# cmusphinx/pocketsphinx

Measured on NVIDIA H100. Metric: frames/sec senone-eval+Viterbi, higher is better.
Workload: dtype f32->i16/i32

## Files before the change

include/psb200.h:

```cpp
#ifndef PSB200_H
#define PSB200_H

#include <stddef.h>
#include <stdint.h>

#ifdef __cplusplus
extern "C" {
#endif

#define PSB_ABI_VERSION 2

typedef enum psb_status_e {
    PSB_OK = 0,
    PSB_ERR_ARG = -1,
    PSB_ERR_CUDA = -2,
    PSB_ERR_NOMEM = -3,
    PSB_ERR_STATE = -4
} psb_status_t;

enum { PSB_KIND_PTM = 0, PSB_KIND_SEMI = 1, PSB_KIND_MS = 2 };

#define PSB_MAX_FEAT 8
#define PSB_MAX_TOPN 8
#define PSB_HMM_MAX_NSTATE 5
// ... 34 lines not shown
int psb_scorer_reset(psb_scorer_t *s);
int psb_scorer_set_frame_idx(psb_scorer_t *s, int32_t frame_idx);
int32_t psb_scorer_get_frame_idx(const psb_scorer_t *s);
int psb_scorer_frame_eval(psb_scorer_t *s, int16_t *senscr, const uint8_t *senone_active,
                          int32_t n_senone_active, const float *const *feat, int32_t frame,
                          int32_t compallsen);

typedef struct psb_batch_s psb_batch_t;

int psb_batch_create(psb_model_t *m, int32_t max_utts, int64_t max_frames, psb_batch_t **out);
void psb_batch_free(psb_batch_t *b);
int psb_batch_score_host(psb_batch_t *b, const float *feats, const int32_t *utt_off,
                         int32_t n_utt, int16_t *senscr);
int psb_batch_score_device(psb_batch_t *b, const float *d_feats, const int32_t *utt_off,
                           int32_t n_utt, int16_t *d_senscr);
int psb_batch_sync(psb_batch_t *b);
int16_t *psb_batch_senscr_device(psb_batch_t *b);
int psb_batch_last_kernel_ms(psb_batch_t *b, float *out3);
int psb_batch_event_record(psb_batch_t *b, int slot);
int psb_batch_event_elapsed_ms(psb_batch_t *b, float *ms);
int psb_batch_tc_check(psb_batch_t *b, float *ratio, int32_t *max_candidates, int64_t *stats4);
#define PSB_TC_N_COUNTERS 15
int psb_batch_tc_counters(psb_batch_t *b, int64_t *out, int32_t n);
#define PSB_MS_PLAN_N 14
int psb_batch_ms_plan(psb_batch_t *b, int64_t total_frames, int64_t *out, int32_t n);
#define PSB_TM_PLAN_N 5
int psb_batch_tm_plan(psb_batch_t *b, int64_t total_frames, int64_t *out, int32_t n);
int psb_batch_get_topn(psb_batch_t *b, int32_t *rec, int64_t n_frames);

typedef struct psb_hmm_s {
    void *ctx;
    int32_t score[PSB_HMM_MAX_NSTATE];
    int32_t history[PSB_HMM_MAX_NSTATE];
    int32_t out_score;
    int32_t out_history;
    uint16_t ssid;
    uint16_t senid[PSB_HMM_MAX_NSTATE];
    int32_t bestscore;
    int16_t tmatid;
    int32_t frame;
    uint8_t mpx;
    uint8_t n_emit_state;
} psb_hmm_t;

typedef struct psb_hmmctx_s psb_hmmctx_t;

// ... 268 lines not shown
```

pocketsphinx_b200/_lib.py:

```python
import ctypes as C
import os

HERE = os.path.dirname(os.path.abspath(__file__))
LIB_PATH = os.path.join(HERE, "libpsb200.so")

MAX_FEAT = 8


class PsbError(RuntimeError):
    pass


class ModelDesc(C.Structure):
    _fields_ = [("kind", C.c_int32), ("n_sen", C.c_int32), ("n_mgau", C.c_int32), ("n_feat", C.c_int32),
                ("n_density", C.c_int32), ("topn", C.c_int32), ("featlen", C.c_int32 * MAX_FEAT),
                ("ds_ratio", C.c_int32), ("aw", C.c_int32), ("logadd_ms_size", C.c_int32),
                ("logadd_ms_zero", C.c_int32), ("on_device", C.c_int32),
                ("mean", C.c_void_p), ("var", C.c_void_p), ("det", C.c_void_p), ("mixw", C.c_void_p),
                ("mixw_cb", C.c_void_p), ("sen2cb", C.c_void_p), ("logadd8", C.c_void_p),
                ("logadd_ms", C.c_void_p), ("topn_beam", C.c_void_p), ("fixed_point", C.c_int32)]


_VP, _I32, _I64 = C.c_void_p, C.c_int32, C.c_int64
class FeDesc(C.Structure):
# ... 56 lines not shown
    ("psb_scorer_get_frame_idx", _I32, [_VP]),
    ("psb_scorer_frame_eval", C.c_int, [_VP, _VP, _VP, _I32, _VP, _I32, _I32]),
    ("psb_batch_create", C.c_int, [_VP, _I32, _I64, C.POINTER(_VP)]),
    ("psb_batch_free", None, [_VP]),
    ("psb_batch_score_host", C.c_int, [_VP, _VP, _VP, _I32, _VP]),
    ("psb_batch_score_device", C.c_int, [_VP, _VP, _VP, _I32, _VP]),
    ("psb_batch_sync", C.c_int, [_VP]),
    ("psb_batch_senscr_device", _VP, [_VP]),
    ("psb_batch_last_kernel_ms", C.c_int, [_VP, _VP]),
    ("psb_batch_get_topn", C.c_int, [_VP, _VP, _I64]),
    ("psb_batch_event_record", C.c_int, [_VP, C.c_int]),
    ("psb_batch_event_elapsed_ms", C.c_int, [_VP, _VP]),
    ("psb_hmmctx_create", C.c_int, [_I32, _VP, _I32, _VP, _I32, _I32, C.c_int, C.POINTER(_VP)]),
    ("psb_hmmctx_free", None, [_VP]),
    ("psb_hmm_vit_eval_batch", C.c_int, [_VP, _VP, _I32, _VP, _VP]),
    ("psb_hmm_vit_eval_ptrs", C.c_int, [_VP, _VP, _I32, _VP, _VP]),
    ("psb_hmmset_create", C.c_int, [_VP, C.c_int64, _I32, C.POINTER(_VP)]),
    ("psb_hmmset_free", None, [_VP]),
    ("psb_hmmset_upload", C.c_int, [_VP, _VP, C.c_int64, _VP, _I32]),
    ("psb_hmmset_download", C.c_int, [_VP, _VP]),
    ("psb_hmmset_eval_frames_device", C.c_int, [_VP, _VP, _VP, _VP, _I32, _VP, C.POINTER(C.c_float)]),
    ("psb_batch_tc_check", C.c_int, [_VP, C.POINTER(C.c_float), C.POINTER(C.c_int32), _VP]),
    ("psb_batch_tc_counters", C.c_int, [_VP, _VP, _I32]),
    ("psb_batch_ms_plan", C.c_int, [_VP, _I64, _VP, _I32]),
    ("psb_batch_tm_plan", C.c_int, [_VP, _I64, _VP, _I32]),
    ("psb_hmmset_use_batch_stream", C.c_int, [_VP, _VP]),
    ("psb_hmmset_snapshot", C.c_int, [_VP]),
    ("psb_hmmset_restore", C.c_int, [_VP]),
    ("psb_hmmset_sweep_device", C.c_int, [_VP, _VP, _I64, _VP, _VP, _I32, _VP, C.POINTER(C.c_float)]),
    ("psb_hmmset_sweep_beam_device", C.c_int, [_VP, _VP, _I64, _VP, _VP, _I32, _I32, _I32, _I32, _VP, _VP, C.POINTER(C.c_float)]),
    ("psb_hmmset_eval_host", C.c_int, [_VP, _VP, _VP]),
    ("psb_allphone_batch_device", C.c_int, [_VP, _VP, _VP, _I32, _I32, _VP, _VP, _VP, _VP, _I32, _I32, _I32, _I32, _VP, _I32, _VP]),
    ("psb_allphone_lm_batch_device", C.c_int, [_VP, _VP, _VP, _I32, _I32, _VP, _VP, _VP, _VP, _I32, _I32, _I32, _I32, _VP, _VP, _VP, _VP, _I32, _VP]),
    ("psb_allphone_net_batch_device", C.c_int, [_VP, _VP, _VP, _I32, _I32, _VP, _VP, _VP, _VP, _VP, _I32, _I32, _I32, _I32, _I32, _VP, _VP, _I32, _VP, _VP, _I32, _VP]),
    ("psb_kws_batch_device", C.c_int, [_VP, _VP, _VP, _I32, _I32, _VP, _VP, _I32, _VP, _VP, _VP, _VP, _I32, _I32, _VP, _I32, _VP]),
    ("psb_fsg_batch_device", C.c_int, [_VP, C.POINTER(FsgDesc), _VP, _VP, _I32, _VP, _I32, _VP]),
    ("psb_ngram_fwdtree_batch_device", C.c_int, [_VP, C.POINTER(NgramDesc), _VP, _VP, _I32, _VP, _I32, _VP, _I32, _VP, _I32, _VP, _VP]),
    ("psb_ngram_fwdflat_batch_device", C.c_int, [_VP, C.POINTER(NgramDesc), _VP, _VP, _I32, _VP, _I32, _VP, _VP, _I32, _VP, _I32, _VP, _VP]),
    ("psb_selftest_block_scan", C.c_int, [C.c_int, _VP, _I32, _VP]),
    ("psb_fsg_find_exit", C.c_int, [_VP, _I32, _VP, _I32, _I32, _I32, _I32, _VP, _VP]),
    ("psb_fsg_backtrace", _I32, [_VP, _I32, _VP, _I32, _I32, _VP, _I32]),
    ("psb_ngram_find_exit", C.c_int, [_VP, _I32, _VP, _I32, _I32, _VP, _VP]),
    ("psb_ngram_backtrace", _I32, [_VP, _I32, _I32, _VP, _I32]),
    ("psb_ngram_segments", _I32, [C.POINTER(NgramDesc), _VP, _I32, _VP, _I32, _I32, C.c_float, _VP, _I32]),
    ("psb_ngram_two_pass_batch_device", C.c_int, [_VP, C.POINTER(NgramDesc), _VP, _VP, _I32, _VP, _I32, _I32, _I32, _VP, _I32, _VP, _I32,
                                                   _VP, _VP, _VP]),
# ... 72 lines not shown
```

pocketsphinx_b200/csrc/psb_ptm_tc.cu:

```cuda
#include "psb_gau.cuh"
#include "psb_internal.cuh"

#include <algorithm>
#include <cmath>
#include <cstring>

namespace {

constexpr int TC_ROWS = 128;
constexpr int TC_K = 32;
constexpr int TC_CAP = 18;
constexpr float TC_ERR = 1.0f / 262144.f;

enum {
    ST_ROWS, ST_FILTER_ALONE, ST_EXACT_DIST, ST_TIE_FLAGS,
    ST_OVER_CAP,
    ST_LANE_OVER,
    ST_FALLBACK_LISTED, ST_FALLBACK_ALL,
    ST_SPLIT,
    ST_FAIL_GAP, ST_FAIL_STRADDLE, ST_FAIL_SIGN, ST_FAIL_SAT,
    ST_N
};
constexpr size_t TC_CHECK_BYTES = 16 + 8 * ST_N;

__device__ __forceinline__ float to_tf32(float x)
{
    unsigned r;
    asm("cvt.rna.tf32.f32 %0, %1;" : "=r"(r) : "f"(x));
    return __uint_as_float(r);
}

struct Top5 {
    int s[5];
    unsigned c;
    int c4;
    int n;
};

__device__ __forceinline__ void top5_insert(Top5 &t, int s, int c)
{
    int p = 0;
#pragma unroll
    for (int j = 0; j < 5; ++j) p += (j < t.n && t.s[j] >= s) ? 1 : 0;
    if (p >= 5) return;
#pragma unroll
    for (int j = 4; j >= 1; --j)
        if (j > p) t.s[j] = t.s[j - 1];
#pragma unroll
    for (int j = 0; j < 5; ++j)
        if (j == p) t.s[j] = s;
    if (p < 4) {
        const unsigned lowmask = p == 0 ? 0u : (0xffffffffu >> (32 - 8 * p));
        t.c4 = (int)(t.c >> 24);
        t.c = (t.c & lowmask) | ((unsigned)c << (8 * p)) | ((t.c << 8) & ~(lowmask | (0xffu << (8 * p))));
    }
    else
        t.c4 = c;
    if (t.n < 5) ++t.n;
}

constexpr int WG_ROWS = 64;
constexpr int WG_SLOTS = (TC_CAP + 1) * WG_ROWS * 4;
constexpr int WG_EXTRA = WG_SLOTS * 8 + WG_ROWS * 4 * 4 + WG_ROWS * 4 + 2 * WG_ROWS * 4 + WG_ROWS * 20;

__device__ __forceinline__ uint64_t wgmma_desc(const void *p, unsigned lbo_bytes, unsigned sbo_bytes)
{
    const uint64_t a = (uint64_t)(((unsigned)__cvta_generic_to_shared(p) >> 4) & 0x3fffu);
    return a | ((uint64_t)((lbo_bytes >> 4) & 0x3fffu) << 16) | ((uint64_t)((sbo_bytes >> 4) & 0x3fffu) << 32);
}

template <int R>
__device__ __forceinline__ void wgmma_fence_regs(float (&d)[R])
{
#pragma unroll
    for (int i = 0; i < R; ++i) asm volatile("" : "+f"(d[i])::"memory");
}

__device__ __forceinline__ void warpgroup_bar(int id) { asm volatile("bar.sync %0, 128;" ::"r"(id) : "memory"); }

template <int N>
struct Wgmma;
#define PSB_ACC8(i) "+f"(d[i]), "+f"(d[i + 1]), "+f"(d[i + 2]), "+f"(d[i + 3]), "+f"(d[i + 4]), "+f"(d[i + 5]), "+f"(d[i + 6]), "+f"(d[i + 7])
template <> struct Wgmma<64> {
    static __device__ __forceinline__ void mma(float (&d)[32], uint64_t a, uint64_t b, int accumulate)
    {
        asm volatile("{\n.reg .pred p;\nsetp.ne.b32 p, %34, 0;\nwgmma.mma_async.sync.aligned.m64n64k8.f32.tf32.tf32 {"
// ... 14 lines not shown
        "}, %64, %65, p, 1, 1;\n}\n"
        : PSB_ACC8(0), PSB_ACC8(8), PSB_ACC8(16), PSB_ACC8(24), PSB_ACC8(32), PSB_ACC8(40), PSB_ACC8(48), PSB_ACC8(56)
        : "l"(a), "l"(b), "r"(accumulate));
    }
};
template <> struct Wgmma<256> {
    static __device__ __forceinline__ void mma(float (&d)[128], uint64_t a, uint64_t b, int accumulate)
    {
        asm volatile("{\n.reg .pred p;\nsetp.ne.b32 p, %130, 0;\nwgmma.mma_async.sync.aligned.m64n256k8.f32.tf32.tf32 {"
        "%0,%1,%2,%3,%4,%5,%6,%7,%8,%9,%10,%11,%12,%13,%14,%15,%16,%17,%18,%19,%20,%21,%22,%23,%24,%25,%26,%27,%28,%29,"
        "%30,%31,%32,%33,%34,%35,%36,%37,%38,%39,%40,%41,%42,%43,%44,%45,%46,%47,%48,%49,%50,%51,%52,%53,%54,%55,%56,"
        "%57,%58,%59,%60,%61,%62,%63,%64,%65,%66,%67,%68,%69,%70,%71,%72,%73,%74,%75,%76,%77,%78,%79,%80,%81,%82,%83,"
        "%84,%85,%86,%87,%88,%89,%90,%91,%92,%93,%94,%95,%96,%97,%98,%99,%100,%101,%102,%103,%104,%105,%106,%107,%108,"
        "%109,%110,%111,%112,%113,%114,%115,%116,%117,%118,%119,%120,%121,%122,%123,%124,%125,%126,%127"
        "}, %128, %129, p, 1, 1;\n}\n"
        : PSB_ACC8(0), PSB_ACC8(8), PSB_ACC8(16), PSB_ACC8(24), PSB_ACC8(32), PSB_ACC8(40), PSB_ACC8(48), PSB_ACC8(56),
          PSB_ACC8(64), PSB_ACC8(72), PSB_ACC8(80), PSB_ACC8(88), PSB_ACC8(96), PSB_ACC8(104), PSB_ACC8(112),
          PSB_ACC8(120)
        : "l"(a), "l"(b), "r"(accumulate));
    }
};
#undef PSB_ACC8

template <int FL, int ND, bool CHECK>
__global__ void __launch_bounds__(2 * 128, 1)
ptm_wgmma_kernel(const float *__restrict__ feats, long long total, int D, const int32_t *__restrict__ featoff,
                 const int32_t *__restrict__ klist, const float *__restrict__ wumma, const float *__restrict__ cen,
                 const float *__restrict__ bnd, const float *__restrict__ rec, const size_t *__restrict__ rec_off,
                 int4 *__restrict__ out, unsigned *__restrict__ flags, long long flag_words, int K, int n_feat,
                 int tiles_per_cta, uint4 *__restrict__ items, unsigned *__restrict__ n_items, unsigned item_cap,
                 float *__restrict__ check, unsigned long long *__restrict__ stats)
{
    constexpr int RF = (1 + 2 * FL + 3) / 4 * 4;
    constexpr int NTL = ND / 8;
    constexpr int NPG = NTL / 8;
    constexpr unsigned FULL = 0xffffffffu;
    static_assert(2 * FL + 1 <= TC_K && (ND == 64 || ND == 128 || ND == 256), "shape");
    extern __shared__ __align__(128) unsigned char wg_smem[];
    const int tid = threadIdx.x, wg = tid >> 7, t = tid & 127, warp = t >> 5, lane = tid & 31;
    float *sW = reinterpret_cast<float *>(wg_smem);
    float *sX = sW + 2 * 8 * ND * 4 + wg * (2 * 8 * WG_ROWS * 4);
    unsigned char *ex = wg_smem + (size_t)2 * 8 * ND * 16 + 2 * (2 * 8 * WG_ROWS * 16) + (size_t)wg * WG_EXTRA;
    float2 *Pv = reinterpret_cast<float2 *>(ex);
    unsigned *Pm = reinterpret_cast<unsigned *>(Pv + WG_SLOTS);
    float *thrs = reinterpret_cast<float *>(Pm + WG_ROWS * 4);
    float *epsr = thrs + WG_ROWS;
    unsigned *Lc = reinterpret_cast<unsigned *>(epsr + 2 * WG_ROWS);

    const int k = klist[blockIdx.x];
    const int f = k % n_feat;
    {
        const float4 *src = reinterpret_cast<const float4 *>(wumma + (size_t)k * 2 * 8 * ND * 4);
        float4 *dst = reinterpret_cast<float4 *>(sW);
        for (int i = tid; i < 2 * 8 * ND; i += 2 * 128) dst[i] = src[i];
    }
    __syncthreads();
    const float *m = cen + (size_t)k * 16, *bb = bnd + (size_t)k * 32;
    const float *rc = rec + rec_off[k];
    const int r = t & (WG_ROWS - 1), half = t >> 6;
    const int g = lane >> 2, q4 = lane & 3;
    const int ra = warp * 16 + g, rb = ra + 8;

    float xn[FL];
    auto fetch = [&](long long row) {
        const float *p = feats + (row < total ? row : 0) * D + featoff[f];
#pragma unroll
        for (int j = 0; j < FL; ++j) xn[j] = row < total ? p[j] : 0.f;
    };
    auto prepare = [&](float *eps) {
        float v[TC_K];
        float S = bb[2 * FL];
#pragma unroll
        for (int j = 0; j < FL; ++j) {
            const float y = __fsub_rn(xn[j], m[j]);
            const float y2 = __fmul_rn(y, y);
            v[j] = y2;
            v[FL + j] = y;
            if (half == 0) {
                S = __fadd_ru(S, __fmul_ru(bb[j], y2));
                S = __fadd_ru(S, __fmul_ru(bb[FL + j], fabsf(y)));
            }
        }
        v[2 * FL] = 1.0f;
#pragma unroll
        for (int j = 2 * FL + 1; j < TC_K; ++j) v[j] = 0.f;
#pragma unroll
        for (int kc = 0; kc < 8; ++kc) {
            if ((kc & 1) != half) continue;
            float4 h, l;
            h.x = to_tf32(v[4 * kc]); h.y = to_tf32(v[4 * kc + 1]); h.z = to_tf32(v[4 * kc + 2]); h.w = to_tf32(v[4 * kc + 3]);
            l.x = to_tf32(__fsub_rn(v[4 * kc], h.x)); l.y = to_tf32(__fsub_rn(v[4 * kc + 1], h.y));
            l.z = to_tf32(__fsub_rn(v[4 * kc + 2], h.z)); l.w = to_tf32(__fsub_rn(v[4 * kc + 3], h.w));
            reinterpret_cast<float4 *>(sX)[kc * WG_ROWS + r] = h;
            reinterpret_cast<float4 *>(sX)[(8 + kc) * WG_ROWS + r] = l;
        }
        if (half == 0) eps[r] = __fadd_ru(__fmul_ru(S, TC_ERR), 2.0f);
        asm volatile("fence.proxy.async.shared::cta;" ::: "memory");
        warpgroup_bar(1 + wg);
    };
    float acc[ND / 2];
    auto gemm = [&]() {
#pragma unroll
        for (int i = 0; i < ND / 2; ++i) acc[i] = 0.f;
        wgmma_fence_regs(acc);
        asm volatile("wgmma.fence.sync.aligned;" ::: "memory");
#pragma unroll
        for (int pass = 0; pass < 3; ++pass) {
            const int ha = pass == 0 ? 1 : 0, hb = pass == 1 ? 1 : 0;
#pragma unroll
            for (int ks = 0; ks < 4; ++ks) {
                const uint64_t ad = wgmma_desc(sX + (size_t)(ha * 8 + 2 * ks) * WG_ROWS * 4, WG_ROWS * 16, 128);
                const uint64_t bd = wgmma_desc(sW + (size_t)(hb * 8 + 2 * ks) * ND * 4, ND * 16, 128);
                Wgmma<ND>::mma(acc, ad, bd, (pass | ks) ? 1 : 0);
            }
        }
        asm volatile("wgmma.commit_group.sync.aligned;" ::: "memory");
    };

    auto resolve = [&](const long long row0, const float *eps) {
        const int rr = t >> 1, h = t & 1;
        const long long row = row0 + rr;
        const bool valid = row < total;
        unsigned char *lb = reinterpret_cast<unsigned char *>(Lc + rr * 5);
        float a[5] = {-INFINITY, -INFINITY, -INFINITY, -INFINITY, -INFINITY};
        int c[5] = {0, 0, 0, 0, 0};
        int nl = 0;
        bool over = false;
        {
            const float thr = thrs[rr];
            auto cand = [&](float v, int col) {
                const bool p = v >= thr;
                if (p && nl < TC_CAP) lb[h ? TC_CAP - 1 - nl : nl] = (unsigned char)col;
                nl += p ? 1 : 0;
                v = p ? v : -INFINITY;
#pragma unroll
                for (int j = 0; j < 5; ++j) {
                    const bool s = v > a[j];
                    const float tv = a[j];
                    const int tc = c[j];
                    a[j] = s ? v : tv; c[j] = s ? col : tc;
                    v = s ? tv : v; col = s ? tc : col;
                }
            };
            unsigned m0 = Pm[rr * 4 + 2 * h], m1 = Pm[rr * 4 + 2 * h + 1];
            over = __popc(m0) > TC_CAP || __popc(m1) > TC_CAP;
            int j0 = 0, j1 = 0;
            while ((m0 | m1) != 0u) {
                const bool first = m0 != 0u;
                const unsigned msk = first ? m0 : m1;
                const int i = __ffs(msk) - 1, q = 2 * h + (first ? 0 : 1), j = first ? j0 : j1;
                const float2 v = Pv[j * WG_ROWS * 4 + rr * 4 + q];
                cand(v.x, 8 * i + 2 * q);
                cand(v.y, 8 * i + 2 * q + 1);
                if (first) { m0 = ++j0 < TC_CAP ? m0 & (m0 - 1u) : 0u; }
                else { m1 = ++j1 < TC_CAP ? m1 & (m1 - 1u) : 0u; }
            }
        }
        const int n1 = __shfl_xor_sync(FULL, nl, 1), n = nl + n1;
        over = __shfl_xor_sync(FULL, (int)over, 1) != 0 || over;
        {
            float b[5];
            int bc[5];
#pragma unroll
            for (int j = 0; j < 5; ++j) { b[j] = __shfl_xor_sync(FULL, a[j], 1); bc[j] = __shfl_xor_sync(FULL, c[j], 1); }
#pragma unroll
// ... 27 lines not shown
                    if (n > TC_CAP) atomicAdd(stats + ST_OVER_CAP, 1ull);
                    if (over) atomicAdd(stats + ST_LANE_OVER, 1ull);
                    if (listed) {
                        if (!gap_ok) atomicAdd(stats + ST_FAIL_GAP, 1ull);
                        if (!straddle_ok) atomicAdd(stats + ST_FAIL_STRADDLE, 1ull);
                        if (!sign_ok) atomicAdd(stats + ST_FAIL_SIGN, 1ull);
                        if (!sat_ok) atomicAdd(stats + ST_FAIL_SAT, 1ull);
                    }
                }
                if (certain) {
                    unsigned cb = 0, eb = 0;
#pragma unroll
                    for (int j = 0; j < 4; ++j) {
                        int ev = qv[0] - qv[j];
                        ev = ev > 255 ? 255 : ev;
                        cb |= (unsigned)c[j] << (8 * j);
                        eb |= (unsigned)ev << (8 * j);
                    }
                    out[row * K + k] = make_int4(qv[0], (int)cb, (int)eb, 0);
                    if (CHECK) { atomicAdd(stats, 1ull); atomicAdd(stats + 1, 1ull); }
                }
            }
        }
        __syncwarp();
        const bool doubt = valid && h == 0 && !certain;
        const int n0 = listed ? nl : 255, nb = listed ? n1 : 0;
        if (CHECK && doubt && listed && nl > 0 && n1 > 0) atomicAdd(stats + ST_SPLIT, 1ull);
        bool handled = false;
        if (items) {
            const unsigned need = __ballot_sync(FULL, doubt);
            if (need) {
                const int leader = __ffs(need) - 1;
                unsigned base = 0;
                if (lane == leader) base = atomicAdd(n_items, (unsigned)__popc(need));
                base = __shfl_sync(FULL, base, leader);
                const unsigned slot = base + (unsigned)__popc(need & ((1u << lane) - 1u));
                if (doubt && slot < item_cap) {
                    const unsigned *w = Lc + rr * 5;
                    items[2 * (size_t)slot] = make_uint4((unsigned)row, (unsigned)k | ((unsigned)n0 << 16) | ((unsigned)nb << 24), w[0], w[1]);
                    items[2 * (size_t)slot + 1] = make_uint4(w[2], w[3], w[4], (unsigned)(row >> 32));
                    handled = true;
                    if (CHECK) atomicAdd(stats, 1ull);
                }
            }
        }
        if (doubt && !handled) {
            float x[FL];
            const float *px = feats + row * D + featoff[f];
#pragma unroll
            for (int j = 0; j < FL; ++j) x[j] = px[j];
            Top5 top;
            top.n = 0; top.c = 0u; top.c4 = 0;
#pragma unroll
            for (int j = 0; j < 5; ++j) top.s[j] = INT_MIN;
            const int cnt_l = listed ? n : ND;
            if (CHECK) atomicAdd(stats + (listed ? ST_FALLBACK_LISTED : ST_FALLBACK_ALL), 1ull);
            for (int i = 0; i < cnt_l; ++i) {
                const int cw = listed ? (int)lb[i < n0 ? i : i - n0 + TC_CAP - nb] : i;
                const float d = gau_dist<FL>(reinterpret_cast<const float4 *>(rc + (size_t)cw * RF), x);
                top5_insert(top, f2i_clamped(d), cw);
            }
            const bool distinct = top.n >= 5 && top.s[0] > top.s[1] && top.s[1] > top.s[2] && top.s[2] > top.s[3] && top.s[3] > top.s[4];
            const int tp = top.s[0] >> PSB_SENSCR_SHIFT;
            unsigned eb = 0;
#pragma unroll
            for (int j = 0; j < 4; ++j) {
                int ev = tp - (top.s[j] >> PSB_SENSCR_SHIFT);
                ev = ev > 255 ? 255 : ev;
                eb |= (unsigned)ev << (8 * j);
            }
            out[row * K + k] = make_int4(tp, (int)top.c, (int)eb, 0);
            if (!distinct) atomicOr(&flags[(size_t)k * flag_words + (row >> 5)], 1u << (row & 31));
            if (CHECK) { atomicAdd(stats, 1ull); atomicAdd(stats + 2, (unsigned long long)cnt_l); if (!distinct) atomicAdd(stats + 3, 1ull); }
        }
    };

    long long row0 = (long long)blockIdx.y * tiles_per_cta * TC_ROWS + wg * WG_ROWS;
    if (row0 >= total) return;
    fetch(row0 + r);
    prepare(epsr);
    int buf = 0;
    for (int tile = 0;; ++tile, buf ^= 1, row0 += TC_ROWS) {
        gemm();
        const bool more = tile + 1 < tiles_per_cta && row0 + TC_ROWS < total;
        if (more) fetch(row0 + TC_ROWS + r);
        if (tile > 0) {
            resolve(row0 - TC_ROWS, epsr + (buf ^ 1) * WG_ROWS);
            warpgroup_bar(1 + wg);
        }
        const float *eps = epsr + buf * WG_ROWS;
        asm volatile("wgmma.wait_group.sync.aligned 0;" ::: "memory");
        wgmma_fence_regs(acc);

        float gma[8], gmb[8];
#pragma unroll
        for (int q = 0; q < 8; ++q) {
            float a = -INFINITY, b = -INFINITY;
#pragma unroll
            for (int i = q * NPG; i < (q + 1) * NPG; ++i) {
                a = fmaxf(fmaxf(a, acc[4 * i]), acc[4 * i + 1]);
                b = fmaxf(fmaxf(b, acc[4 * i + 2]), acc[4 * i + 3]);
            }
            a = fmaxf(a, __shfl_xor_sync(FULL, a, 1)); a = fmaxf(a, __shfl_xor_sync(FULL, a, 2));
            b = fmaxf(b, __shfl_xor_sync(FULL, b, 1)); b = fmaxf(b, __shfl_xor_sync(FULL, b, 2));
            gma[q] = a; gmb[q] = b;
        }
        auto fifth = [](float (&gm)[8]) {
            auto cmpx = [&](int i, int j) { const float hi = fmaxf(gm[i], gm[j]); gm[j] = fminf(gm[i], gm[j]); gm[i] = hi; };
#pragma unroll
            for (int o = 0; o < 8; o += 4) { cmpx(o, o + 1); cmpx(o + 2, o + 3); cmpx(o, o + 2); cmpx(o + 1, o + 3); cmpx(o + 1, o + 2); }
            return fmaxf(fmaxf(fminf(gm[0], gm[7]), fminf(gm[1], gm[6])), fmaxf(fminf(gm[2], gm[5]), fminf(gm[3], gm[4])));
        };
        const float e_a = eps[ra], e_b = eps[rb];
        const float thra = __fsub_rd(__fsub_rd(floorf(__fsub_rd(fifth(gma), e_a)), 1.0f), e_a);
        const float thrb = __fsub_rd(__fsub_rd(floorf(__fsub_rd(fifth(gmb), e_b)), 1.0f), e_b);
        {
            constexpr int SS = WG_ROWS * 4;
            int oa = ra * 4 + q4, ob = rb * 4 + q4;
            const int lim_a = oa + TC_CAP * SS, lim_b = ob + TC_CAP * SS;
            unsigned ma = 0u, mb = 0u;
#pragma unroll
            for (int i = 0; i < NTL; ++i) {
                const bool pa = fmaxf(acc[4 * i], acc[4 * i + 1]) >= thra;
                const bool pb = fmaxf(acc[4 * i + 2], acc[4 * i + 3]) >= thrb;
                if (pa) Pv[oa] = make_float2(acc[4 * i], acc[4 * i + 1]);
                if (pb) Pv[ob] = make_float2(acc[4 * i + 2], acc[4 * i + 3]);
                oa = pa ? min(oa + SS, lim_a) : oa;
                ob = pb ? min(ob + SS, lim_b) : ob;
                ma |= pa ? 1u << i : 0u;
                mb |= pb ? 1u << i : 0u;
            }
            Pm[ra * 4 + q4] = ma;
            Pm[rb * 4 + q4] = mb;
            if (q4 == 0) { thrs[ra] = thra; thrs[rb] = thrb; }
        }
        if (CHECK) {
            float worst = 0.f;
#pragma unroll
            for (int h = 0; h < 2; ++h) {
                const int rr = h ? rb : ra;
                if (row0 + rr >= total) continue;
                const float *px = feats + (row0 + rr) * D + featoff[f];
                const float er = eps[rr];
#pragma unroll
                for (int i = 0; i < NTL; ++i)
#pragma unroll
                    for (int e = 0; e < 2; ++e) {
                        const float *rp = rc + (size_t)(8 * i + 2 * q4 + e) * RF;
                        float d = rp[0];
                        for (int j = 0; j < FL; ++j) {
                            const float df = __fsub_rn(px[j], rp[1 + 2 * j]);
                            d = __fsub_rn(d, __fmul_rn(__fmul_rn(df, df), rp[2 + 2 * j]));
                        }
                        worst = fmaxf(worst, __fdividef(fabsf(acc[4 * i + 2 * h + e] - d), er));
                    }
            }
            atomicMax(reinterpret_cast<int *>(check), __float_as_int(worst));
        }
        warpgroup_bar(1 + wg);
        if (!more) break;
        prepare(epsr + (buf ^ 1) * WG_ROWS);
    }
    resolve(row0, epsr + buf * WG_ROWS);
}

template <int FL>
__global__ void __launch_bounds__(128)
ptm_tc_exact_kernel(const float *__restrict__ feats, int D, const int32_t *__restrict__ featoff, const uint4 *__restrict__ items,
                    const unsigned *__restrict__ n_items, unsigned item_cap, const float *__restrict__ rec,
                    const size_t *__restrict__ rec_off, int4 *__restrict__ out, unsigned *__restrict__ flags, long long flag_words,
                    int K, int n_feat, int nd, unsigned long long *__restrict__ stats)
{
    constexpr int RF = (1 + 2 * FL + 3) / 4 * 4;
    const unsigned count = min(*n_items, item_cap);
    for (unsigned i = blockIdx.x * blockDim.x + threadIdx.x; i < count; i += gridDim.x * blockDim.x) {
        const uint4 a = items[2 * (size_t)i], b = items[2 * (size_t)i + 1];
        const long long row = (long long)a.x | ((long long)b.w << 32);
        const int k = (int)(a.y & 0xffffu), n0 = (int)((a.y >> 16) & 0xffu), n1 = (int)(a.y >> 24);
        const unsigned wv[5] = {a.z, a.w, b.x, b.y, b.z};
        const float *px = feats + row * D + featoff[k % n_feat];
        const float *rc = rec + rec_off[k];
        float x[FL];
#pragma unroll
        for (int j = 0; j < FL; ++j) x[j] = px[j];
        Top5 top;
        top.n = 0; top.c = 0u; top.c4 = 0;
#pragma unroll
        for (int j = 0; j < 5; ++j) top.s[j] = INT_MIN;
        const int cnt = n0 == 255 ? nd : n0 + n1;
        for (int q = 0; q < cnt; ++q) {
            const int pos = q < n0 ? q : q - n0 + TC_CAP - n1;
            const int cw = n0 == 255 ? q : (int)((wv[pos >> 2] >> (8 * (pos & 3))) & 0xffu);
            const float d = gau_dist<FL>(reinterpret_cast<const float4 *>(rc + (size_t)cw * RF), x);
            top5_insert(top, f2i_clamped(d), cw);
        }
        const bool distinct = top.n >= 5 && top.s[0] > top.s[1] && top.s[1] > top.s[2] && top.s[2] > top.s[3] && top.s[3] > top.s[4];
        const int tp = top.s[0] >> PSB_SENSCR_SHIFT;
        unsigned eb = 0;
#pragma unroll
// ... 101 lines not shown
                        eb |= (unsigned)ev << (8 * j);
                    }
                    out[row * K + k] = make_int4(tp, (int)cb, (int)eb, 0);
                }
                __syncwarp();
            }
        }
    }
}

float round_tf32_host(float x)
{
    uint32_t u;
    memcpy(&u, &x, 4);
    if ((u & 0x7f800000u) == 0x7f800000u) return x;
    u = (u + 0x1000u) & ~0x1fffu;
    float r;
    memcpy(&r, &u, 4);
    return r;
}

template <int FL, int ND>
int launch_wgmma(psb_batch_t *b, const float *d_feats, long long total, const int32_t *d_klist, int n_k, const int32_t *d_featoff,
               bool check)
{
    psb_model_t *m = b->m;
    const size_t smem = (size_t)2 * 8 * ND * 16 + 2 * ((size_t)2 * 8 * WG_ROWS * 16 + WG_EXTRA);
    const long long tiles = (total + TC_ROWS - 1) / TC_ROWS;
    const int n_sm = psb_sm_count(m->device);
    int per_sm = 1;
    PSB_CUDA(cudaFuncSetAttribute(ptm_wgmma_kernel<FL, ND, false>, cudaFuncAttributeMaxDynamicSharedMemorySize, (int)smem));
    PSB_CUDA(cudaOccupancyMaxActiveBlocksPerMultiprocessor(&per_sm, ptm_wgmma_kernel<FL, ND, false>, TC_ROWS * 2, smem));
    int tpc = 1;
    while (tpc < 32 && (tiles / (tpc * 2)) * n_k >= (long long)n_sm * std::max(per_sm, 1) * 4) tpc *= 2;
    PSB_REQUIRE((tiles + tpc - 1) / tpc <= 65535, "too many frames for one launch of the tensor-core filter");
    const dim3 grid((unsigned)n_k, (unsigned)((tiles + tpc - 1) / tpc));
    b->tc_last_tpc = tpc;
    b->tc_last_ctas = grid.y;
    float *chk = b->d_tc_check;
    unsigned long long *stats = reinterpret_cast<unsigned long long *>(b->d_tc_check + 4);
    if (check) {
        auto kern = ptm_wgmma_kernel<FL, ND, true>;
        PSB_CUDA(cudaFuncSetAttribute(kern, cudaFuncAttributeMaxDynamicSharedMemorySize, (int)smem));
        kern<<<grid, TC_ROWS * 2, smem, b->stream>>>(d_feats, total, m->sumlen, d_featoff, d_klist, m->d_tc_wumma, m->d_tc_cen, m->d_tc_bnd,
                                                m->d_rec, m->d_rec_off, b->d_topn, b->d_tc_flags, (long long)b->tc_flag_words, m->K,
                                                m->n_feat, tpc, b->d_tc_items, b->d_tc_nitems, b->tc_item_cap, chk, stats);
    }
    else {
        auto kern = ptm_wgmma_kernel<FL, ND, false>;
        PSB_CUDA(cudaFuncSetAttribute(kern, cudaFuncAttributeMaxDynamicSharedMemorySize, (int)smem));
        kern<<<grid, TC_ROWS * 2, smem, b->stream>>>(d_feats, total, m->sumlen, d_featoff, d_klist, m->d_tc_wumma, m->d_tc_cen, m->d_tc_bnd,
                                                m->d_rec, m->d_rec_off, b->d_topn, b->d_tc_flags, (long long)b->tc_flag_words, m->K,
                                                m->n_feat, tpc, b->d_tc_items, b->d_tc_nitems, b->tc_item_cap, nullptr, nullptr);
    }
    PSB_LAUNCH_CHECK();
    if (b->d_tc_items) {
        const unsigned blocks = (unsigned)std::min<size_t>(((size_t)b->tc_item_cap + 127) / 128, (size_t)n_sm * 64);
        ptm_tc_exact_kernel<FL><<<blocks, 128, 0, b->stream>>>(d_feats, m->sumlen, d_featoff, b->d_tc_items, b->d_tc_nitems, b->tc_item_cap,
                                                              m->d_rec, m->d_rec_off, b->d_topn, b->d_tc_flags, (long long)b->tc_flag_words,
                                                              m->K, m->n_feat, ND, check ? stats : nullptr);
        PSB_LAUNCH_CHECK();
    }
    return PSB_OK;
}

}

int psb_tc_prepare(psb_model_t *m, const float *hm, const float *hv, const float *hd)
{
    m->tc_ok = false;
    if (m->kind != PSB_KIND_PTM || m->fixed_point || m->topn != 4) return PSB_OK;
    if (m->n_density != 64 && m->n_density != 128 && m->n_density != 256) return PSB_OK;
// ... 47 lines not shown
    if (!rc) rc = m->d_tc_bnd.reserve(bnd.size());
    if (rc) return rc;
    PSB_CUDA(cudaMemcpy(m->d_tc_wumma, wu.data(), wu.size() * sizeof(float), cudaMemcpyHostToDevice));
    PSB_CUDA(cudaMemcpy(m->d_tc_cen, cen.data(), cen.size() * sizeof(float), cudaMemcpyHostToDevice));
    PSB_CUDA(cudaMemcpy(m->d_tc_bnd, bnd.data(), bnd.size() * sizeof(float), cudaMemcpyHostToDevice));
    m->tc_ok = true;
    return PSB_OK;
}

bool psb_tc_usable(const psb_model_t *m)
{
    return m->tc_ok && m->ds_ratio == 1;
}

int psb_launch_ptm_tc(psb_batch_t *b, const float *d_feats, const int32_t *utt_off, int32_t n_utt, const int32_t *d_klist,
                      const int32_t *d_featoff)
{
    psb_model_t *m = b->m;
    const long long total = utt_off[n_utt];
    const size_t fw = (size_t)((total + 31) / 32) + 1;
    int rc = b->d_tc_flags.reserve(fw * m->K, fw * m->K / 8);
    if (!rc) rc = b->d_uttoff.reserve((size_t)n_utt + 1, 64);
    if (!rc && !b->d_tc_check) {
        rc = b->d_tc_check.reserve(TC_CHECK_BYTES / sizeof(float));
        if (!rc) PSB_CUDA(cudaMemsetAsync(b->d_tc_check, 0, TC_CHECK_BYTES, b->stream));
    }
    if (!rc) rc = b->d_tc_nitems.reserve(1);
    if (rc) return rc;
    {
        const size_t want = std::max<size_t>(4096, (size_t)total * m->K / 4);
        if (want > b->tc_item_cap) {
            const unsigned cap = (unsigned)std::min<size_t>(want + want / 8, 0x7fffffffu);
            b->tc_item_cap = 0;
            if ((rc = b->d_tc_items.reserve(2 * (size_t)cap))) return rc;
            b->tc_item_cap = cap;
        }
        PSB_CUDA(cudaMemsetAsync(b->d_tc_nitems, 0, 4, b->stream));
    }
    b->tc_flag_words = fw;
    PSB_CUDA(cudaMemsetAsync(b->d_tc_flags, 0, fw * m->K * 4, b->stream));
    PSB_CUDA(cudaMemcpyAsync(b->d_uttoff, utt_off, ((size_t)n_utt + 1) * sizeof(int32_t), cudaMemcpyHostToDevice, b->stream));
    static const bool check = [] { const char *v = getenv("PSB_TC_CHECK"); return v && atoi(v) != 0; }();
    switch (m->n_density) {
    case 256: rc = launch_wgmma<13, 256>(b, d_feats, total, d_klist, m->K, d_featoff, check); break;
    case 128: rc = launch_wgmma<13, 128>(b, d_feats, total, d_klist, m->K, d_featoff, check); break;
    default: rc = launch_wgmma<13, 64>(b, d_feats, total, d_klist, m->K, d_featoff, check); break;
    }
    if (rc) return rc;
    const long long chains = (long long)n_utt * m->K;
    const unsigned blocks = (unsigned)((chains * 32 + 127) / 128);
#define PSB_FIXW(NDW) ptm_fixup_warp_kernel<13, NDW><<<blocks, 128, 0, b->stream>>>(d_feats, m->sumlen, d_featoff, b->d_uttoff, n_utt, \
        m->d_rec, m->d_rec_off, b->d_topn, b->d_tc_flags, (long long)fw, m->K, m->n_feat)
    if (m->n_density == 256) PSB_FIXW(8);
    else if (m->n_density == 128) PSB_FIXW(4);
    else PSB_FIXW(2);
#undef PSB_FIXW
    PSB_LAUNCH_CHECK();
    return PSB_OK;
}

extern "C" int psb_batch_tc_check(psb_batch_t *b, float *ratio, int32_t *max_candidates, int64_t *stats4)
{
    PSB_REQUIRE(b && ratio && max_candidates, "psb_batch_tc_check: null argument");
    *ratio = 0.f; *max_candidates = 0;
    if (stats4) stats4[0] = stats4[1] = stats4[2] = stats4[3] = 0;
    if (!b->d_tc_check) return PSB_OK;
    PSB_CUDA(cudaSetDevice(b->m->device));
    PSB_CUDA(cudaStreamSynchronize(b->stream));
    unsigned char h[64];
    PSB_CUDA(cudaMemcpy(h, b->d_tc_check, sizeof(h), cudaMemcpyDeviceToHost));
    memcpy(ratio, h, 4);
    memcpy(max_candidates, h + 4, 4);
    if (stats4) memcpy(stats4, h + 16, 32);
    return PSB_OK;
}

extern "C" int psb_batch_tc_counters(psb_batch_t *b, int64_t *out, int32_t n)
{
    PSB_REQUIRE(b && (out || n == 0) && n >= 0, "psb_batch_tc_counters: bad argument");
    static_assert(ST_N + 2 == PSB_TC_N_COUNTERS, "psb200.h lists every counter");
    int64_t v[PSB_TC_N_COUNTERS] = {0};
    if (b->d_tc_check) {
        PSB_CUDA(cudaSetDevice(b->m->device));
        PSB_CUDA(cudaStreamSynchronize(b->stream));
        PSB_CUDA(cudaMemcpy(v, reinterpret_cast<unsigned char *>(b->d_tc_check.get()) + 16, 8 * ST_N, cudaMemcpyDeviceToHost));
    }
    v[ST_N] = b->tc_last_tpc;
    v[ST_N + 1] = b->tc_last_ctas;
    memcpy(out, v, sizeof(int64_t) * (size_t)std::min<int32_t>(n, PSB_TC_N_COUNTERS));
    return PSB_OK;
}
```

Baseline: 12.80 million.

## Defer fallback item pushes, chunk item reservations, and add per-phase cycle timing

Each warp now reserves fallback-item slots from the global counter in chunks of 32 instead of one atomic per resolve. The item writes and inline fallback scoring are deferred to the next tile's pass so they overlap the following GEMM, and leftover reserved slots are marked as holes that the consumer kernel skips. It also reorganises the bound sum into a tree reduction, replaces the sequential top-5 insertion with a compare-all select, and adds an optional clock-based phase profiler behind an environment variable. The cost is a bit more shared memory and code complexity, plus possible hole entries in the item list.

After: 12.97 million (median of 6 runs). +1.3%, better.

```diff
diff --git a/include/psb200.h b/include/psb200.h
--- a/include/psb200.h
+++ b/include/psb200.h
@@ -80,6 +80,8 @@
 int psb_batch_tc_check(psb_batch_t *b, float *ratio, int32_t *max_candidates, int64_t *stats4);
 #define PSB_TC_N_COUNTERS 15
 int psb_batch_tc_counters(psb_batch_t *b, int64_t *out, int32_t n);
+#define PSB_TC_N_PHASES 9
+int psb_batch_tc_phase_cycles(psb_batch_t *b, int64_t *out, int32_t n);
 #define PSB_MS_PLAN_N 14
 int psb_batch_ms_plan(psb_batch_t *b, int64_t total_frames, int64_t *out, int32_t n);
 #define PSB_TM_PLAN_N 5
diff --git a/pocketsphinx_b200/_lib.py b/pocketsphinx_b200/_lib.py
--- a/pocketsphinx_b200/_lib.py
+++ b/pocketsphinx_b200/_lib.py
@@ -102,6 +102,7 @@
     ("psb_hmmset_eval_frames_device", C.c_int, [_VP, _VP, _VP, _VP, _I32, _VP, C.POINTER(C.c_float)]),
     ("psb_batch_tc_check", C.c_int, [_VP, C.POINTER(C.c_float), C.POINTER(C.c_int32), _VP]),
     ("psb_batch_tc_counters", C.c_int, [_VP, _VP, _I32]),
+    ("psb_batch_tc_phase_cycles", C.c_int, [_VP, _VP, _I32]),
     ("psb_batch_ms_plan", C.c_int, [_VP, _I64, _VP, _I32]),
     ("psb_batch_tm_plan", C.c_int, [_VP, _I64, _VP, _I32]),
     ("psb_hmmset_use_batch_stream", C.c_int, [_VP, _VP]),
diff --git a/pocketsphinx_b200/csrc/psb_ptm_tc.cu b/pocketsphinx_b200/csrc/psb_ptm_tc.cu
--- a/pocketsphinx_b200/csrc/psb_ptm_tc.cu
+++ b/pocketsphinx_b200/csrc/psb_ptm_tc.cu
@@ -23,6 +23,20 @@
 };
 constexpr size_t TC_CHECK_BYTES = 16 + 8 * ST_N;
 
+enum {
+    PH_STAGE,
+    PH_PREP,
+    PH_ISSUE, PH_WAIT,
+    PH_MAXIMA,
+    PH_STORE,
+    PH_RESOLVE,
+    PH_PUSH,
+    PH_BAR,
+    PH_N
+};
+static_assert(PH_N == PSB_TC_N_PHASES, "psb200.h lists every phase");
+constexpr size_t TC_DEBUG_BYTES = TC_CHECK_BYTES + 8 * PH_N;
+
 __device__ __forceinline__ float to_tf32(float x)
 {
     unsigned r;
@@ -60,8 +74,10 @@
 }
 
 constexpr int WG_ROWS = 64;
+constexpr unsigned TC_CHUNK = 32;
+constexpr unsigned TC_HOLE = 0xffffffffu;
 constexpr int WG_SLOTS = (TC_CAP + 1) * WG_ROWS * 4;
-constexpr int WG_EXTRA = WG_SLOTS * 8 + WG_ROWS * 4 * 4 + WG_ROWS * 4 + 2 * WG_ROWS * 4 + WG_ROWS * 20;
+constexpr int WG_EXTRA = WG_SLOTS * 8 + WG_ROWS * 4 * 4 + WG_ROWS * 4 + 2 * WG_ROWS * 4 + WG_ROWS * 20 + WG_ROWS * 4;
 
 __device__ __forceinline__ uint64_t wgmma_desc(const void *p, unsigned lbo_bytes, unsigned sbo_bytes)
 {
@@ -122,7 +138,7 @@
 };
 #undef PSB_ACC8
 
-template <int FL, int ND, bool CHECK>
+template <int FL, int ND, bool CHECK, bool TIME>
 __global__ void __launch_bounds__(2 * 128, 1)
 ptm_wgmma_kernel(const float *__restrict__ feats, long long total, int D, const int32_t *__restrict__ featoff,
                  const int32_t *__restrict__ klist, const float *__restrict__ wumma, const float *__restrict__ cen,
@@ -146,6 +162,27 @@
     float *thrs = reinterpret_cast<float *>(Pm + WG_ROWS * 4);
     float *epsr = thrs + WG_ROWS;
     unsigned *Lc = reinterpret_cast<unsigned *>(epsr + 2 * WG_ROWS);
+    unsigned *Ln = Lc + WG_ROWS * 5;
+    unsigned long long *tph = reinterpret_cast<unsigned long long *>(wg_smem + (size_t)2 * 8 * ND * 16 + 2 * (2 * 8 * WG_ROWS * 16 + WG_EXTRA)) +
+                              (tid >> 5) * PH_N;
+    unsigned tl = 0;
+    auto mark = [&](int p) {
+        if (TIME) {
+            const unsigned now = (unsigned)clock();
+            if (lane == 0) tph[p] += now - tl;
+            tl = now;
+        }
+    };
+    auto flush = [&]() {
+        if (TIME) {
+            __syncwarp();
+            if (lane < PH_N) atomicAdd(stats + ST_N + lane, tph[lane]);
+        }
+    };
+    if (TIME) {
+        if (lane < PH_N) tph[lane] = 0ull;
+        tl = (unsigned)clock();
+    }
 
     const int k = klist[blockIdx.x];
     const int f = k % n_feat;
@@ -155,6 +192,7 @@
         for (int i = tid; i < 2 * 8 * ND; i += 2 * 128) dst[i] = src[i];
     }
     __syncthreads();
+    mark(PH_STAGE);
     const float *m = cen + (size_t)k * 16, *bb = bnd + (size_t)k * 32;
     const float *rc = rec + rec_off[k];
     const int r = t & (WG_ROWS - 1), half = t >> 6;
@@ -169,17 +207,26 @@
     };
     auto prepare = [&](float *eps) {
         float v[TC_K];
-        float S = bb[2 * FL];
 #pragma unroll
         for (int j = 0; j < FL; ++j) {
             const float y = __fsub_rn(xn[j], m[j]);
-            const float y2 = __fmul_rn(y, y);
-            v[j] = y2;
+            v[j] = __fmul_rn(y, y);
             v[FL + j] = y;
-            if (half == 0) {
-                S = __fadd_ru(S, __fmul_ru(bb[j], y2));
-                S = __fadd_ru(S, __fmul_ru(bb[FL + j], fabsf(y)));
-            }
+        }
+        float S = 0.f;
+        if (half == 0) {
+            float s[2 * FL + 1];
+#pragma unroll
+            for (int j = 0; j < FL; ++j) {
+                s[j] = __fmul_ru(bb[j], v[j]);
+                s[FL + j] = __fmul_ru(bb[FL + j], fabsf(v[FL + j]));
+            }
+            s[2 * FL] = bb[2 * FL];
+#pragma unroll
+            for (int w = 1; w < 2 * FL + 1; w *= 2)
+#pragma unroll
+                for (int i = 0; i + w < 2 * FL + 1; i += 2 * w) s[i] = __fadd_ru(s[i], s[i + w]);
+            S = s[0];
         }
         v[2 * FL] = 1.0f;
 #pragma unroll
@@ -196,7 +243,9 @@
         }
         if (half == 0) eps[r] = __fadd_ru(__fmul_ru(S, TC_ERR), 2.0f);
         asm volatile("fence.proxy.async.shared::cta;" ::: "memory");
+        mark(PH_PREP);
         warpgroup_bar(1 + wg);
+        mark(PH_BAR);
     };
     float acc[ND / 2];
     auto gemm = [&]() {
@@ -217,6 +266,15 @@
         asm volatile("wgmma.commit_group.sync.aligned;" ::: "memory");
     };
 
+    unsigned res_base = 0u, res_left = 0u;
+    unsigned pend_need = 0u, pend_old = 0u, pend_split = 0u, pend_new = 0u;
+    bool pend_run = false;
+    long long pend_row0 = 0;
+    auto close_run = [&]() {
+        if (items)
+            for (unsigned i = lane; i < res_left; i += 32)
+                if (res_base + i < item_cap) items[2 * (size_t)(res_base + i)] = make_uint4(0u, TC_HOLE, 0u, 0u);
+    };
     auto resolve = [&](const long long row0, const float *eps) {
         const int rr = t >> 1, h = t & 1;
         const long long row = row0 + rr;
@@ -233,14 +291,16 @@
                 if (p && nl < TC_CAP) lb[h ? TC_CAP - 1 - nl : nl] = (unsigned char)col;
                 nl += p ? 1 : 0;
                 v = p ? v : -INFINITY;
-#pragma unroll
-                for (int j = 0; j < 5; ++j) {
-                    const bool s = v > a[j];
-                    const float tv = a[j];
-                    const int tc = c[j];
-                    a[j] = s ? v : tv; c[j] = s ? col : tc;
-                    v = s ? tv : v; col = s ? tc : col;
+                bool gt[5];
+#pragma unroll
+                for (int j = 0; j < 5; ++j) gt[j] = v > a[j];
+#pragma unroll
+                for (int j = 4; j >= 1; --j) {
+                    a[j] = gt[j] ? (gt[j - 1] ? a[j - 1] : v) : a[j];
+                    c[j] = gt[j] ? (gt[j - 1] ? c[j - 1] : col) : c[j];
                 }
+                a[0] = gt[0] ? v : a[0];
+                c[0] = gt[0] ? col : c[0];
             };
             unsigned m0 = Pm[rr * 4 + 2 * h], m1 = Pm[rr * 4 + 2 * h + 1];
             over = __popc(m0) > TC_CAP || __popc(m1) > TC_CAP;
@@ -314,75 +374,105 @@
                 }
             }
         }
+        mark(PH_RESOLVE);
+        const bool doubt = valid && h == 0 && !certain;
+        if (CHECK && doubt && listed && nl > 0 && n1 > 0) atomicAdd(stats + ST_SPLIT, 1ull);
+        if (doubt) Ln[rr] = (unsigned)(listed ? nl : 255) | (unsigned)(listed ? n1 : 0) << 8;
+        pend_need = __ballot_sync(FULL, doubt);
+        pend_row0 = row0;
+        const unsigned cnt = (unsigned)__popc(pend_need);
+        pend_old = res_base;
+        pend_split = min(cnt, res_left);
+        pend_run = cnt > res_left;
+        if (pend_run) {
+            if (items && lane == 0) pend_new = atomicAdd(n_items, TC_CHUNK);
+            res_left = res_left + TC_CHUNK - cnt;
+        }
+        else {
+            res_base += cnt;
+            res_left -= cnt;
+        }
+        mark(PH_PUSH);
+    };
+    auto push_items = [&]() {
+        if (!pend_need) return;
+        const unsigned cnt = (unsigned)__popc(pend_need);
+        unsigned nb0 = 0;
+        if (pend_run) {
+            nb0 = __shfl_sync(FULL, pend_new, 0);
+            res_base = nb0 + (cnt - pend_split);
+        }
         __syncwarp();
-        const bool doubt = valid && h == 0 && !certain;
-        const int n0 = listed ? nl : 255, nb = listed ? n1 : 0;
-        if (CHECK && doubt && listed && nl > 0 && n1 > 0) atomicAdd(stats + ST_SPLIT, 1ull);
-        bool handled = false;
-        if (items) {
-            const unsigned need = __ballot_sync(FULL, doubt);
-            if (need) {
-                const int leader = __ffs(need) - 1;
-                unsigned base = 0;
-                if (lane == leader) base = atomicAdd(n_items, (unsigned)__popc(need));
-                base = __shfl_sync(FULL, base, leader);
-                const unsigned slot = base + (unsigned)__popc(need & ((1u << lane) - 1u));
-                if (doubt && slot < item_cap) {
-                    const unsigned *w = Lc + rr * 5;
-                    items[2 * (size_t)slot] = make_uint4((unsigned)row, (unsigned)k | ((unsigned)n0 << 16) | ((unsigned)nb << 24), w[0], w[1]);
-                    items[2 * (size_t)slot + 1] = make_uint4(w[2], w[3], w[4], (unsigned)(row >> 32));
-                    handled = true;
-                    if (CHECK) atomicAdd(stats, 1ull);
+        if ((pend_need >> lane) & 1u) {
+            const int rr = t >> 1;
+            const long long row = pend_row0 + rr;
+            const unsigned ln = Ln[rr];
+            const int n0 = (int)(ln & 0xffu), nb = (int)(ln >> 8);
+            const bool listed = n0 != 255;
+            const unsigned j = (unsigned)__popc(pend_need & ((1u << lane) - 1u));
+            const unsigned slot = j < pend_split ? pend_old + j : nb0 + (j - pend_split);
+            if (items && slot < item_cap) {
+                const unsigned *w = Lc + rr * 5;
+                items[2 * (size_t)slot] = make_uint4((unsigned)row, (unsigned)k | ((unsigned)n0 << 16) | ((unsigned)nb << 24), w[0], w[1]);
+                items[2 * (size_t)slot + 1] = make_uint4(w[2], w[3], w[4], (unsigned)(row >> 32));
+                if (CHECK) atomicAdd(stats, 1ull);
+            }
+            else {
+                const unsigned char *lb = reinterpret_cast<const unsigned char *>(Lc + rr * 5);
+                float x[FL];
+                const float *px = feats + row * D + featoff[f];
+#pragma unroll
+                for (int j = 0; j < FL; ++j) x[j] = px[j];
+                Top5 top;
+                top.n = 0; top.c = 0u; top.c4 = 0;
+#pragma unroll
+                for (int j = 0; j < 5; ++j) top.s[j] = INT_MIN;
+                const int cnt_l = listed ? n0 + nb : ND;
+                if (CHECK) atomicAdd(stats + (listed ? ST_FALLBACK_LISTED : ST_FALLBACK_ALL), 1ull);
+                for (int i = 0; i < cnt_l; ++i) {
+                    const int cw = listed ? (int)lb[i < n0 ? i : i - n0 + TC_CAP - nb] : i;
+                    const float d = gau_dist<FL>(reinterpret_cast<const float4 *>(rc + (size_t)cw * RF), x);
+                    top5_insert(top, f2i_clamped(d), cw);
                 }
-            }
-        }
-        if (doubt && !handled) {
-            float x[FL];
-            const float *px = feats + row * D + featoff[f];
-#pragma unroll
-            for (int j = 0; j < FL; ++j) x[j] = px[j];
-            Top5 top;
-            top.n = 0; top.c = 0u; top.c4 = 0;
-#pragma unroll
-            for (int j = 0; j < 5; ++j) top.s[j] = INT_MIN;
-            const int cnt_l = listed ? n : ND;
-            if (CHECK) atomicAdd(stats + (listed ? ST_FALLBACK_LISTED : ST_FALLBACK_ALL), 1ull);
-            for (int i = 0; i < cnt_l; ++i) {
-                const int cw = listed ? (int)lb[i < n0 ? i : i - n0 + TC_CAP - nb] : i;
-                const float d = gau_dist<FL>(reinterpret_cast<const float4 *>(rc + (size_t)cw * RF), x);
-                top5_insert(top, f2i_clamped(d), cw);
-            }
-            const bool distinct = top.n >= 5 && top.s[0] > top.s[1] && top.s[1] > top.s[2] && top.s[2] > top.s[3] && top.s[3] > top.s[4];
-            const int tp = top.s[0] >> PSB_SENSCR_SHIFT;
-            unsigned eb = 0;
-#pragma unroll
-            for (int j = 0; j < 4; ++j) {
-                int ev = tp - (top.s[j] >> PSB_SENSCR_SHIFT);
-                ev = ev > 255 ? 255 : ev;
-                eb |= (unsigned)ev << (8 * j);
-            }
-            out[row * K + k] = make_int4(tp, (int)top.c, (int)eb, 0);
-            if (!distinct) atomicOr(&flags[(size_t)k * flag_words + (row >> 5)], 1u << (row & 31));
-            if (CHECK) { atomicAdd(stats, 1ull); atomicAdd(stats + 2, (unsigned long long)cnt_l); if (!distinct) atomicAdd(stats + 3, 1ull); }
-        }
+                const bool distinct = top.n >= 5 && top.s[0] > top.s[1] && top.s[1] > top.s[2] && top.s[2] > top.s[3] && top.s[3] > top.s[4];
+                const int tp = top.s[0] >> PSB_SENSCR_SHIFT;
+                unsigned eb = 0;
+#pragma unroll
+                for (int j = 0; j < 4; ++j) {
+                    int ev = tp - (top.s[j] >> PSB_SENSCR_SHIFT);
+                    ev = ev > 255 ? 255 : ev;
+                    eb |= (unsigned)ev << (8 * j);
+                }
+                out[row * K + k] = make_int4(tp, (int)top.c, (int)eb, 0);
+                if (!distinct) atomicOr(&flags[(size_t)k * flag_words + (row >> 5)], 1u << (row & 31));
+                if (CHECK) { atomicAdd(stats, 1ull); atomicAdd(stats + 2, (unsigned long long)cnt_l); if (!distinct) atomicAdd(stats + 3, 1ull); }
+            }
+        }
+        pend_need = 0u;
+        __syncwarp();
+        mark(PH_PUSH);
     };
 
     long long row0 = (long long)blockIdx.y * tiles_per_cta * TC_ROWS + wg * WG_ROWS;
-    if (row0 >= total) return;
+    if (row0 >= total) { flush(); return; }
     fetch(row0 + r);
     prepare(epsr);
     int buf = 0;
     for (int tile = 0;; ++tile, buf ^= 1, row0 += TC_ROWS) {
         gemm();
+        mark(PH_ISSUE);
         const bool more = tile + 1 < tiles_per_cta && row0 + TC_ROWS < total;
         if (more) fetch(row0 + TC_ROWS + r);
         if (tile > 0) {
+            push_items();
             resolve(row0 - TC_ROWS, epsr + (buf ^ 1) * WG_ROWS);
             warpgroup_bar(1 + wg);
+            mark(PH_BAR);
         }
         const float *eps = epsr + buf * WG_ROWS;
         asm volatile("wgmma.wait_group.sync.aligned 0;" ::: "memory");
         wgmma_fence_regs(acc);
+        mark(PH_WAIT);
 
         float gma[8], gmb[8];
 #pragma unroll
@@ -406,6 +496,7 @@
         const float e_a = eps[ra], e_b = eps[rb];
         const float thra = __fsub_rd(__fsub_rd(floorf(__fsub_rd(fifth(gma), e_a)), 1.0f), e_a);
         const float thrb = __fsub_rd(__fsub_rd(floorf(__fsub_rd(fifth(gmb), e_b)), 1.0f), e_b);
+        mark(PH_MAXIMA);
         {
             constexpr int SS = WG_ROWS * 4;
             int oa = ra * 4 + q4, ob = rb * 4 + q4;
@@ -426,6 +517,7 @@
             Pm[rb * 4 + q4] = mb;
             if (q4 == 0) { thrs[ra] = thra; thrs[rb] = thrb; }
         }
+        mark(PH_STORE);
         if (CHECK) {
             float worst = 0.f;
 #pragma unroll
@@ -450,10 +542,15 @@
             atomicMax(reinterpret_cast<int *>(check), __float_as_int(worst));
         }
         warpgroup_bar(1 + wg);
+        mark(PH_BAR);
         if (!more) break;
         prepare(epsr + (buf ^ 1) * WG_ROWS);
     }
+    push_items();
     resolve(row0, epsr + buf * WG_ROWS);
+    push_items();
+    close_run();
+    flush();
 }
 
 template <int FL>
@@ -466,7 +563,9 @@
     constexpr int RF = (1 + 2 * FL + 3) / 4 * 4;
     const unsigned count = min(*n_items, item_cap);
     for (unsigned i = blockIdx.x * blockDim.x + threadIdx.x; i < count; i += gridDim.x * blockDim.x) {
-        const uint4 a = items[2 * (size_t)i], b = items[2 * (size_t)i + 1];
+        const uint4 a = items[2 * (size_t)i];
+        if (a.y == TC_HOLE) continue;
+        const uint4 b = items[2 * (size_t)i + 1];
         const long long row = (long long)a.x | ((long long)b.w << 32);
         const int k = (int)(a.y & 0xffffu), n0 = (int)((a.y >> 16) & 0xffu), n1 = (int)(a.y >> 24);
         const unsigned wv[5] = {a.z, a.w, b.x, b.y, b.z};
@@ -614,15 +713,15 @@
 
 template <int FL, int ND>
 int launch_wgmma(psb_batch_t *b, const float *d_feats, long long total, const int32_t *d_klist, int n_k, const int32_t *d_featoff,
-               bool check)
+               bool check, bool time)
 {
     psb_model_t *m = b->m;
     const size_t smem = (size_t)2 * 8 * ND * 16 + 2 * ((size_t)2 * 8 * WG_ROWS * 16 + WG_EXTRA);
     const long long tiles = (total + TC_ROWS - 1) / TC_ROWS;
     const int n_sm = psb_sm_count(m->device);
     int per_sm = 1;
-    PSB_CUDA(cudaFuncSetAttribute(ptm_wgmma_kernel<FL, ND, false>, cudaFuncAttributeMaxDynamicSharedMemorySize, (int)smem));
-    PSB_CUDA(cudaOccupancyMaxActiveBlocksPerMultiprocessor(&per_sm, ptm_wgmma_kernel<FL, ND, false>, TC_ROWS * 2, smem));
+    PSB_CUDA(cudaFuncSetAttribute(ptm_wgmma_kernel<FL, ND, false, false>, cudaFuncAttributeMaxDynamicSharedMemorySize, (int)smem));
+    PSB_CUDA(cudaOccupancyMaxActiveBlocksPerMultiprocessor(&per_sm, ptm_wgmma_kernel<FL, ND, false, false>, TC_ROWS * 2, smem));
     int tpc = 1;
     while (tpc < 32 && (tiles / (tpc * 2)) * n_k >= (long long)n_sm * std::max(per_sm, 1) * 4) tpc *= 2;
     PSB_REQUIRE((tiles + tpc - 1) / tpc <= 65535, "too many frames for one launch of the tensor-core filter");
@@ -631,15 +730,23 @@
     b->tc_last_ctas = grid.y;
     float *chk = b->d_tc_check;
     unsigned long long *stats = reinterpret_cast<unsigned long long *>(b->d_tc_check + 4);
-    if (check) {
-        auto kern = ptm_wgmma_kernel<FL, ND, true>;
+    if (time) {
+        auto kern = ptm_wgmma_kernel<FL, ND, false, true>;
+        const size_t smem_t = smem + 8 * PH_N * 8;
+        PSB_CUDA(cudaFuncSetAttribute(kern, cudaFuncAttributeMaxDynamicSharedMemorySize, (int)smem_t));
+        kern<<<grid, TC_ROWS * 2, smem_t, b->stream>>>(d_feats, total, m->sumlen, d_featoff, d_klist, m->d_tc_wumma, m->d_tc_cen,
+                                                  m->d_tc_bnd, m->d_rec, m->d_rec_off, b->d_topn, b->d_tc_flags, (long long)b->tc_flag_words,
+                                                  m->K, m->n_feat, tpc, b->d_tc_items, b->d_tc_nitems, b->tc_item_cap, nullptr, stats);
+    }
+    else if (check) {
+        auto kern = ptm_wgmma_kernel<FL, ND, true, false>;
         PSB_CUDA(cudaFuncSetAttribute(kern, cudaFuncAttributeMaxDynamicSharedMemorySize, (int)smem));
         kern<<<grid, TC_ROWS * 2, smem, b->stream>>>(d_feats, total, m->sumlen, d_featoff, d_klist, m->d_tc_wumma, m->d_tc_cen, m->d_tc_bnd,
                                                 m->d_rec, m->d_rec_off, b->d_topn, b->d_tc_flags, (long long)b->tc_flag_words, m->K,
                                                 m->n_feat, tpc, b->d_tc_items, b->d_tc_nitems, b->tc_item_cap, chk, stats);
     }
     else {
-        auto kern = ptm_wgmma_kernel<FL, ND, false>;
+        auto kern = ptm_wgmma_kernel<FL, ND, false, false>;
         PSB_CUDA(cudaFuncSetAttribute(kern, cudaFuncAttributeMaxDynamicSharedMemorySize, (int)smem));
         kern<<<grid, TC_ROWS * 2, smem, b->stream>>>(d_feats, total, m->sumlen, d_featoff, d_klist, m->d_tc_wumma, m->d_tc_cen, m->d_tc_bnd,
                                                 m->d_rec, m->d_rec_off, b->d_topn, b->d_tc_flags, (long long)b->tc_flag_words, m->K,
@@ -733,8 +840,8 @@
     int rc = b->d_tc_flags.reserve(fw * m->K, fw * m->K / 8);
     if (!rc) rc = b->d_uttoff.reserve((size_t)n_utt + 1, 64);
     if (!rc && !b->d_tc_check) {
-        rc = b->d_tc_check.reserve(TC_CHECK_BYTES / sizeof(float));
-        if (!rc) PSB_CUDA(cudaMemsetAsync(b->d_tc_check, 0, TC_CHECK_BYTES, b->stream));
+        rc = b->d_tc_check.reserve(TC_DEBUG_BYTES / sizeof(float));
+        if (!rc) PSB_CUDA(cudaMemsetAsync(b->d_tc_check, 0, TC_DEBUG_BYTES, b->stream));
     }
     if (!rc) rc = b->d_tc_nitems.reserve(1);
     if (rc) return rc;
@@ -752,10 +859,11 @@
     PSB_CUDA(cudaMemsetAsync(b->d_tc_flags, 0, fw * m->K * 4, b->stream));
     PSB_CUDA(cudaMemcpyAsync(b->d_uttoff, utt_off, ((size_t)n_utt + 1) * sizeof(int32_t), cudaMemcpyHostToDevice, b->stream));
     static const bool check = [] { const char *v = getenv("PSB_TC_CHECK"); return v && atoi(v) != 0; }();
+    static const bool time = [] { const char *v = getenv("PSB_TC_TIME"); return v && atoi(v) != 0; }();
     switch (m->n_density) {
-    case 256: rc = launch_wgmma<13, 256>(b, d_feats, total, d_klist, m->K, d_featoff, check); break;
-    case 128: rc = launch_wgmma<13, 128>(b, d_feats, total, d_klist, m->K, d_featoff, check); break;
-    default: rc = launch_wgmma<13, 64>(b, d_feats, total, d_klist, m->K, d_featoff, check); break;
+    case 256: rc = launch_wgmma<13, 256>(b, d_feats, total, d_klist, m->K, d_featoff, check, time); break;
+    case 128: rc = launch_wgmma<13, 128>(b, d_feats, total, d_klist, m->K, d_featoff, check, time); break;
+    default: rc = launch_wgmma<13, 64>(b, d_feats, total, d_klist, m->K, d_featoff, check, time); break;
     }
     if (rc) return rc;
     const long long chains = (long long)n_utt * m->K;
@@ -801,3 +909,17 @@
     memcpy(out, v, sizeof(int64_t) * (size_t)std::min<int32_t>(n, PSB_TC_N_COUNTERS));
     return PSB_OK;
 }
+
+extern "C" int psb_batch_tc_phase_cycles(psb_batch_t *b, int64_t *out, int32_t n)
+{
+    PSB_REQUIRE(b && (out || n == 0) && n >= 0, "psb_batch_tc_phase_cycles: bad argument");
+    int64_t v[PSB_TC_N_PHASES] = {0};
+    if (b->d_tc_check) {
+        PSB_CUDA(cudaSetDevice(b->m->device));
+        PSB_CUDA(cudaStreamSynchronize(b->stream));
+        PSB_CUDA(cudaMemcpy(v, reinterpret_cast<unsigned char *>(b->d_tc_check.get()) + TC_CHECK_BYTES, 8 * PH_N,
+                            cudaMemcpyDeviceToHost));
+    }
+    memcpy(out, v, sizeof(int64_t) * (size_t)std::min<int32_t>(n, PSB_TC_N_PHASES));
+    return PSB_OK;
+}
```
